# ZhiHuangHn/vtkCloudPoint

Hardware: AMD Instinct MI355X
Metric: Mpoints/s DBSCAN+label @10M pts (higher is better)
Workload: dtype f64; 1 GPU; C4: 10000000-pt cloud (half uniform background, 200 Gaussian blobs), one monolithic DBImproved.dbscan, metric L1_2D, eps 0.1, minPts 10; mode=single, points_total=10000000, points_per_gpu=10000000, clusters=27380, resident_in_hbm=True

## Files before the change

### vtkcloudpoint_amd/csrc/gridbuild.hip

```cpp
#include <algorithm>
#include <mutex>
#include <unordered_map>

#include "grid_common.hpp"

using namespace vcpg;

namespace {

constexpr int PT = 1024;
constexpr int PCH_MIN = 8192;
constexpr int FT = 1024;
constexpr uint32_t MAXB = 8192;
constexpr uint32_t wcap(int) { return 4096u; }
constexpr uint32_t QUEUE_FROM = 32;

typedef float4 Rec;

template <int GD>
__device__ __forceinline__ Rec rec_make(const float* qf, uint32_t idx, uint32_t cell) {
  return GD == 2 ? make_float4(qf[0], qf[1], __uint_as_float(idx), __uint_as_float(cell))
                 : make_float4(qf[0], qf[1], qf[2], __uint_as_float(idx));
}
template <int GD>
__device__ __forceinline__ uint32_t rec_cell(const Rec& r, const GridP& g, uint32_t& idx) {
  if (GD == 2) {
    idx = __float_as_uint(r.z);
    return __float_as_uint(r.w);
  }
  idx = __float_as_uint(r.w);
  const float qf[3] = {r.x, r.y, r.z};
  int cc[3];
  return cell_of32<3>(qf, g, cc);
}

template <int GD>
__device__ __forceinline__ uint32_t point_cell(const double* __restrict__ c, int64_t i, int stride, const GridP& g, float* qf) {
  double q[3];
  int cc[3];
  load_in<GD>(c, i, stride, q);
#pragma unroll
  for (int a = 0; a < GD; a++) qf[a] = rel32(q[a], g.mn[a], g.scale);
  return cell_of32<GD>(qf, g, cc);
}

struct PartGeom {
  uint32_t csh;
  uint32_t B;
  uint32_t a;
  uint32_t NS;
  uint32_t chunk;
  uint32_t nchunk;
};

inline int env_int(const char* name, int dflt, int lo, int hi) {
  const char* e = getenv(name);
  int v = e ? atoi(e) : dflt;
  return v < lo ? lo : v > hi ? hi : v;
}

inline PartGeom part_geom(int64_t n, uint32_t ncells) {
  static const int csh_max = env_int("VCP_CPB_LOG2", 14, 10, 14);
  static const int target = env_int("VCP_PART_CHUNKS", 256, 64, 8192);
  PartGeom p;
  int csh = csh_max;
  while (csh > 10 && ((uint64_t)ncells >> csh) * 4096ull < (uint64_t)n) csh--;
  p.csh = (uint32_t)csh;
  p.B = (uint32_t)((((uint64_t)ncells + 1) + ((1ull << p.csh) - 1)) >> p.csh);
  p.a = 0;
  while (((p.B + (1u << p.a) - 1u) >> p.a) > MAXB) p.a++;
  p.NS = (p.B + (1u << p.a) - 1u) >> p.a;
  int64_t chunk = (n + target - 1) / target;
  if (chunk < PCH_MIN) chunk = PCH_MIN;
  chunk = (chunk + PT - 1) / PT * PT;
  p.chunk = (uint32_t)chunk;
  p.nchunk = (uint32_t)((n + chunk - 1) / chunk);
  return p;
}

template <int GD, bool GROUPED>
__global__ __launch_bounds__(PT) void k_part_hist(const double* __restrict__ c, int64_t n, int stride, GridP g,
                                                 const int32_t* __restrict__ group, int glo, int ghi, uint32_t csh,
                                                 uint32_t B, uint32_t chunk, uint32_t nchunk,
                                                 uint32_t* __restrict__ counts, uint32_t* __restrict__ qcount,
                                                 uint32_t* __restrict__ ctcount) {
  extern __shared__ uint32_t h[];
  if (blockIdx.x == 0 && threadIdx.x == 0) {
    *qcount = 0u;
    ctcount[0] = 0u;
  }
  for (uint32_t k = threadIdx.x; k < B; k += PT) h[k] = 0;
  __syncthreads();
  const int64_t first = (int64_t)blockIdx.x * chunk;
  const int64_t last = min(first + (int64_t)chunk, n);
#pragma unroll 4
  for (int64_t i = first + threadIdx.x; i < last; i += PT) {
    if (GROUPED) {
      const int gg = group[i];
      if (gg < glo || gg >= ghi) continue;
    }
    float qf[3];
    atomicAdd(&h[point_cell<GD>(c, i, stride, g, qf) >> csh], 1u);
  }
  __syncthreads();
  for (uint32_t k = threadIdx.x; k < B; k += PT) counts[(size_t)k * nchunk + blockIdx.x] = h[k];
}

template <int GD, bool GROUPED>
__global__ __launch_bounds__(PT) void k_part_scatter(const double* __restrict__ c, int64_t n, int stride, GridP g,
                                                    const int32_t* __restrict__ group, int glo, int ghi, uint32_t csh,
                                                    uint32_t B, uint32_t chunk, uint32_t nchunk,
                                                    const uint32_t* __restrict__ base, Rec* __restrict__ rec,
                                                    uint32_t* __restrict__ pos) {
  extern __shared__ uint32_t h[];
  for (uint32_t k = threadIdx.x; k < B; k += PT) h[k] = base[(size_t)k * nchunk + blockIdx.x];
  __syncthreads();
  const int64_t first = (int64_t)blockIdx.x * chunk;
  const int64_t last = min(first + (int64_t)chunk, n);
#pragma unroll 4
  for (int64_t i = first + threadIdx.x; i < last; i += PT) {
    if (GROUPED) {
      const int gg = group[i];
      if (gg < glo || gg >= ghi) {
        if (pos) pos[i] = NONE;
        continue;
      }
    }
    float qf[3];
    const uint32_t cell = point_cell<GD>(c, i, stride, g, qf);
    rec[atomicAdd(&h[cell >> csh], 1u)] = rec_make<GD>(qf, (uint32_t)i, cell);
  }
}

__device__ __forceinline__ uint32_t padded(uint32_t i) { return i + (i >> 5); }

template <int GD, bool GROUPED, int NT = FT>
__device__ __forceinline__ void fine_flush(uint32_t s0, uint32_t m, const float* s32, const uint32_t* sidx,
                                           const uint32_t* __restrict__ ord, const uint8_t* __restrict__ in_classed,
                                           const int32_t* __restrict__ group, float* __restrict__ sorted32,
                                           uint32_t* __restrict__ sord, uint32_t* __restrict__ sidx_out,
                                           int32_t* __restrict__ sgroup, uint8_t* __restrict__ flags,
                                           uint32_t* __restrict__ pos) {
  if (GD == 2) {
    const float2* src = reinterpret_cast<const float2*>(s32);
    float2* dst = reinterpret_cast<float2*>(sorted32) + s0;
    for (uint32_t k = threadIdx.x; k < m; k += NT) dst[k] = src[k];
  } else {
    const float4* src = reinterpret_cast<const float4*>(s32);
    float4* dst = reinterpret_cast<float4*>(sorted32) + s0;
    for (uint32_t k = threadIdx.x; k < m; k += NT) dst[k] = src[k];
  }
  for (uint32_t k = threadIdx.x; k < m; k += NT) {
    const uint32_t i = sidx[k], p = s0 + k;
    sord[p] = ord ? ord[i] : i;
    if (sidx_out) sidx_out[p] = i;
    if (GROUPED) sgroup[p] = group[i];
    if (in_classed) flags[p] = in_classed[i] ? F_CLASSED : 0;
    if (pos) pos[i] = p;
  }
}

template <int GD>
__device__ __forceinline__ void stage_put(float* s32, uint32_t* sidx, uint32_t p, const Rec& r, uint32_t idx) {
  if (GD == 2) reinterpret_cast<float2*>(s32)[p] = make_float2(r.x, r.y);
  else reinterpret_cast<float4*>(s32)[p] = make_float4(r.x, r.y, r.z, 0.0f);
  sidx[p] = idx;
}

__device__ __forceinline__ void bucket_range(const uint32_t* __restrict__ bstart, uint32_t bstride, const uint32_t* __restrict__ total,
                                             uint32_t b, uint32_t B, uint32_t& s, uint32_t& e) {
  s = bstart[(size_t)b * bstride];
  e = (b + 1 < B) ? bstart[(size_t)(b + 1) * bstride] : *total;
}

template <int GD>
__global__ __launch_bounds__(FT) void k_part_split(const Rec* __restrict__ rec, Rec* __restrict__ rec2,
                                                  const uint32_t* __restrict__ base, const uint32_t* __restrict__ total,
                                                  uint32_t nchunk, uint32_t NS, uint32_t a, uint32_t csh, uint32_t B, GridP g,
                                                  uint32_t* __restrict__ bstart) {
  __shared__ uint32_t h[32];
  const uint32_t S = blockIdx.x;
  uint32_t s, e;
  bucket_range(base, nchunk, total, S, NS, s, e);
  const uint32_t subm = (1u << a) - 1u;
  if (threadIdx.x < 32) h[threadIdx.x] = 0u;
  __syncthreads();
  for (uint32_t j = s + threadIdx.x; j < e; j += FT) {
    uint32_t i;
    atomicAdd(&h[(rec_cell<GD>(rec[j], g, i) >> csh) & subm], 1u);
  }
  __syncthreads();
  if (threadIdx.x < 32) {
    const uint32_t v = h[threadIdx.x];
    uint32_t inc = v;
#pragma unroll
    for (int d = 1; d < 32; d <<= 1) {
      const uint32_t t = __shfl_up(inc, d, 64);
      if ((int)threadIdx.x >= d) inc += t;
    }
    const uint32_t first = s + inc - v;
    h[threadIdx.x] = first;
    const uint32_t bk = (S << a) + threadIdx.x;
    if (threadIdx.x <= subm && bk <= B) bstart[bk] = first;
  }
  __syncthreads();
  for (uint32_t j = s + threadIdx.x; j < e; j += FT) {
    const Rec r = rec[j];
    uint32_t i;
    rec2[atomicAdd(&h[(rec_cell<GD>(r, g, i) >> csh) & subm], 1u)] = r;
  }
}

constexpr int FS = 512;
constexpr uint32_t scap(int gd) { return gd == 2 ? 2048u : 1536u; }
constexpr uint32_t SPOP = 128;

template <int GD, bool GROUPED>
__global__ __launch_bounds__(FS) void k_part_fine_small(const Rec* __restrict__ rec, const uint32_t* __restrict__ bstart,
                                                       uint32_t bstride, const uint32_t* __restrict__ total, uint32_t B,
                                                       uint32_t csh, GridP g, const uint32_t* __restrict__ ord,
                                                       const uint8_t* __restrict__ in_classed, const int32_t* __restrict__ group,
                                                       uint4* __restrict__ ctwords, uint32_t* __restrict__ ctdense,
                                                       uint32_t* __restrict__ ctcount, uint8_t* __restrict__ bstate,
                                                       float* __restrict__ sorted32, uint32_t* __restrict__ sord,
                                                       uint32_t* __restrict__ sidx_out, int32_t* __restrict__ sgroup,
                                                       uint8_t* __restrict__ flags, uint32_t* __restrict__ pos) {
  constexpr uint32_t FPR = GD == 2 ? 2 : 4;
  constexpr uint32_t SCAP = scap(GD);
  constexpr int SRPT = SCAP / FS;
  __shared__ uint32_t ws[512 + 2];
  __shared__ uint32_t wlo[512], whi[512];
  __shared__ uint16_t wpi[512];
  __shared__ uint8_t sci[SCAP];
  __shared__ __attribute__((aligned(16))) uint16_t st32[SPOP][32];
  __shared__ __attribute__((aligned(16))) float s32[SCAP * FPR];
  __shared__ uint32_t sidx[SCAP];
  __shared__ uint32_t wsum[FS / 64];
  __shared__ uint32_t s_np, s_dbase;
  const uint32_t b = blockIdx.x;
  uint32_t s, e;
  bucket_range(bstart, bstride, total, b, B, s, e);
  const uint32_t m = e - s;
  if (b + 1 == B && threadIdx.x == 0) ctcount[1] = *total;
  if (m > SCAP) {
    if (threadIdx.x == 0) bstate[b] = 1;
    return;
  }
  const uint32_t CPB = 1u << csh, NW = CPB >> 5, c0 = b << csh;
  const int lane = threadIdx.x & 63, w = threadIdx.x >> 6;
  for (uint32_t k = threadIdx.x; k < NW + 1; k += FS) ws[k] = 0u;
  __syncthreads();
  Rec r[SRPT];
  uint32_t idx[SRPT], lw[SRPT], ci[SRPT], rnk[SRPT];
#pragma unroll
  for (int k = 0; k < SRPT; k++) {
    const uint32_t j = s + (uint32_t)k * FS + threadIdx.x;
    lw[k] = NONE;
    if (j < e) {
      r[k] = rec[j];
      const uint32_t c = rec_cell<GD>(r[k], g, idx[k]) - c0;
      lw[k] = c >> 5;
      ci[k] = c & 31u;
      rnk[k] = atomicAdd(&ws[lw[k]], 1u);
    }
  }
  __syncthreads();
  {
    const uint32_t v = threadIdx.x < NW ? ws[threadIdx.x] : 0u;
    uint32_t inc = v;
#pragma unroll
    for (int d = 1; d < 64; d <<= 1) {
      const uint32_t t = __shfl_up(inc, d, 64);
      if (lane >= d) inc += t;
    }
    if (lane == 63) wsum[w] = inc;
    __syncthreads();
    uint32_t pre = inc - v;
    for (int k = 0; k < w; k++) pre += wsum[k];
    if (threadIdx.x < NW) ws[threadIdx.x] = s + pre;
    if (threadIdx.x == 0) ws[NW] = e;
  }
  __syncthreads();
#pragma unroll
  for (int k = 0; k < SRPT; k++)
    if (lw[k] != NONE) sci[ws[lw[k]] - s + rnk[k]] = (uint8_t)ci[k];
  __syncthreads();
  bool popl = false;
  uint32_t lo = 0u, hi = 0u;
  if (threadIdx.x < NW) {
    const uint32_t a = ws[threadIdx.x] - s, k = ws[threadIdx.x + 1] - s - a;
    if (k > 64u) {
      popl = true;
    } else {
      for (uint32_t i = 0; i < k; i++) {
        const uint32_t bit = 1u << sci[a + i];
        if (lo & hi & bit) continue;
        if (lo & bit) hi ^= bit;
        lo ^= bit;
      }
      popl = (lo & hi) != 0u;
    }
  }
  {
    const unsigned long long dm = __ballot(popl);
    if (lane == 0) wsum[w] = (uint32_t)__popcll(dm);
    __syncthreads();
    uint32_t before = (uint32_t)__popcll(dm & ((1ull << lane) - 1ull)), tot = 0;
    for (int k = 0; k < FS / 64; k++) {
      if (k < w) before += wsum[k];
      tot += wsum[k];
    }
    if (threadIdx.x == 0) s_np = tot;
    if (threadIdx.x < NW) wpi[threadIdx.x] = popl ? (uint16_t)before : (uint16_t)0xFFFFu;
  }
  __syncthreads();
  const uint32_t np = s_np;
  if (np > SPOP) {
    if (threadIdx.x == 0) bstate[b] = 1;
    return;
  }
  if (threadIdx.x == 0) {
    bstate[b] = 0;
    s_dbase = np ? atomicAdd(&ctcount[0], np) : 0u;
  }
  for (uint32_t k = threadIdx.x; k < np * 16u; k += FS) reinterpret_cast<uint32_t*>(&st32[0][0])[k] = 0u;
  if (threadIdx.x < NW && !popl) {
    wlo[threadIdx.x] = lo;
    whi[threadIdx.x] = hi;
  }
  __syncthreads();
#pragma unroll
  for (int k = 0; k < SRPT; k++)
    if (lw[k] != NONE && wpi[lw[k]] != 0xFFFFu) {
      uint16_t* c = &st32[wpi[lw[k]]][ci[k]];
      atomicAdd(reinterpret_cast<uint32_t*>(reinterpret_cast<uintptr_t>(c) & ~(uintptr_t)3), ((uintptr_t)c & 2) ? 0x10000u : 1u);
    }
  __syncthreads();
  {
    const uint32_t hw = threadIdx.x >> 5, li = threadIdx.x & 31u;
    for (uint32_t wd = hw; wd < NW; wd += FS / 32) {
      const uint32_t pi = wpi[wd];
      if (pi == 0xFFFFu) continue;
      const uint32_t c = st32[pi][li];
      uint32_t inc = c;
#pragma unroll
      for (int d = 1; d < 32; d <<= 1) {
        const uint32_t t = __shfl_up(inc, d, 32);
        if ((int)li >= d) inc += t;
      }
      const uint32_t first = ws[wd] + inc - c;
      st32[pi][li] = (uint16_t)(first - s);
      ctdense[(size_t)(s_dbase + pi) * 32u + li] = first;
      const uint32_t cs = min(c, 3u);
      const unsigned long long blo = __ballot(cs & 1u), bhi = __ballot(cs >> 1);
      const int sh = (threadIdx.x & 32) ? 32 : 0;
      if (li == 0) {
        wlo[wd] = (uint32_t)(blo >> sh);
        whi[wd] = (uint32_t)(bhi >> sh);
      }
    }
  }
  __syncthreads();
#pragma unroll
  for (int k = 0; k < SRPT; k++) {
    if (lw[k] == NONE) continue;
    const uint32_t pi = wpi[lw[k]];
    uint32_t p;
    if (pi != 0xFFFFu) {
      uint16_t* c = &st32[pi][ci[k]];
      const bool up = ((uintptr_t)c & 2) != 0;
      const uint32_t old = atomicAdd(reinterpret_cast<uint32_t*>(reinterpret_cast<uintptr_t>(c) & ~(uintptr_t)3), up ? 0x10000u : 1u);
      p = up ? old >> 16 : old & 0xFFFFu;
    } else {
      const uint32_t l = wlo[lw[k]], h = whi[lw[k]], below = (1u << ci[k]) - 1u;
      const uint32_t a = ws[lw[k]] - s;
      p = a + (uint32_t)__popc(l & below) + 2u * (uint32_t)__popc(h & below);
      if ((h >> ci[k]) & 1u)
        for (uint32_t i = 0; i < rnk[k]; i++) p += sci[a + i] == (uint8_t)ci[k] ? 1u : 0u;
    }
    stage_put<GD>(s32, sidx, p, r[k], idx[k]);
  }
  if (threadIdx.x < NW) {
    const size_t W = (size_t)(c0 >> 5) + threadIdx.x;
    const uint32_t pi = wpi[threadIdx.x];
    if (W < vcp_ct_words(g.ncells))
      ctwords[W] = make_uint4(wlo[threadIdx.x], whi[threadIdx.x], ws[threadIdx.x], pi != 0xFFFFu ? s_dbase + pi : NONE);
  }
  __syncthreads();
  fine_flush<GD, GROUPED, FS>(s, m, s32, sidx, ord, in_classed, group, sorted32, sord, sidx_out, sgroup, flags, pos);
}

template <int GD, bool GROUPED>
__global__ __launch_bounds__(FT) void k_part_fine(const Rec* __restrict__ rec, uint32_t* __restrict__ rk,
                                                 const uint32_t* __restrict__ bstart, uint32_t bstride,
                                                 const uint32_t* __restrict__ total, uint32_t B, uint32_t csh, GridP g,
                                                 const uint32_t* __restrict__ ord, const uint8_t* __restrict__ in_classed,
                                                 const int32_t* __restrict__ group, uint4* __restrict__ ctwords,
                                                 uint32_t* __restrict__ ctdense, uint32_t* __restrict__ ctcount,
                                                 float* __restrict__ sorted32, uint32_t* __restrict__ sord,
                                                 uint32_t* __restrict__ sidx_out, int32_t* __restrict__ sgroup,
                                                 uint8_t* __restrict__ flags, uint32_t* __restrict__ pos,
                                                 uint2* __restrict__ queue, uint32_t* __restrict__ qcount,
                                                 const uint8_t* __restrict__ bstate) {
  extern __shared__ __attribute__((aligned(16))) unsigned char lds[];
  __shared__ uint32_t wsum[FT / 64];
  __shared__ uint32_t w_lo[512], w_hi[512], w_slot[512];
  __shared__ uint32_t s_dbase;
  const uint32_t b = blockIdx.x;
  if (bstate[b] == 0) return;
  constexpr uint32_t WCAP = wcap(GD);
  constexpr uint32_t FPR = GD == 2 ? 2 : 4;
  const uint32_t CPB = 1u << csh;
  uint32_t* cnt = reinterpret_cast<uint32_t*>(lds);
  float* s32 = reinterpret_cast<float*>(lds + (((size_t)padded(CPB) + 4) & ~3ull) * 4);
  uint32_t* sidx = reinterpret_cast<uint32_t*>(s32 + (size_t)WCAP * FPR);
  const uint32_t c0 = b << csh;
  uint32_t s, e;
  bucket_range(bstart, bstride, total, b, B, s, e);
  const uint32_t m = e - s;
  const bool big = m > WCAP;
  for (uint32_t k = threadIdx.x; k < padded(CPB); k += FT) cnt[k] = 0;
  __syncthreads();
  for (uint32_t j = s + threadIdx.x; j < e; j += FT) {
    uint32_t i;
    uint32_t* slot = &cnt[padded(rec_cell<GD>(rec[j], g, i) - c0)];
    if (big) rk[j] = atomicAdd(slot, 1u);
    else atomicAdd(slot, 1u);
  }
  __syncthreads();
  const uint32_t PER = CPB / FT;
  const uint32_t first = threadIdx.x * PER;
  uint32_t loc = 0;
  for (uint32_t k = 0; k < PER; k++) loc += cnt[padded(first + k)];
  const int lane = threadIdx.x & 63, w = threadIdx.x >> 6;
  uint32_t inc = loc;
#pragma unroll
  for (int d = 1; d < 64; d <<= 1) {
    const uint32_t t = __shfl_up(inc, d, 64);
    if (lane >= d) inc += t;
  }
  if (lane == 63) wsum[w] = inc;
  __syncthreads();
  uint32_t pre = s + inc - loc;
  for (int k = 0; k < w; k++) pre += wsum[k];
  const uint32_t NW = CPB >> 5;
  uint32_t plo = 0u, phi = 0u;
  const uint32_t wstart = pre;
  {
    const uint32_t bit0 = first & 31u;
    for (uint32_t k = 0; k < PER; k++) {
      const uint32_t v = cnt[padded(first + k)];
      cnt[padded(first + k)] = pre;
      pre += v;
      const uint32_t c = min(v, 3u);
      plo |= (c & 1u) << (bit0 + k);
      phi |= (c >> 1) << (bit0 + k);
    }
    for (uint32_t d = 1; d < 32u / PER; d <<= 1) {
      plo |= (uint32_t)__shfl_xor((int)plo, (int)d, 64);
      phi |= (uint32_t)__shfl_xor((int)phi, (int)d, 64);
    }
    if ((first & 31u) == 0u) {
      w_lo[first >> 5] = plo;
      w_hi[first >> 5] = phi;
      w_slot[first >> 5] = wstart;
    }
  }
  __syncthreads();
  {
    const bool popl = threadIdx.x < NW && (w_lo[threadIdx.x] & w_hi[threadIdx.x]) != 0u;
    const unsigned long long dm = __ballot(popl);
    if (lane == 0) wsum[w] = (uint32_t)__popcll(dm);
    __syncthreads();
    uint32_t before = (uint32_t)__popcll(dm & ((1ull << lane) - 1ull)), tot = 0;
    for (int k = 0; k < FT / 64; k++) {
      if (k < w) before += wsum[k];
      tot += wsum[k];
    }
    if (threadIdx.x == 0) s_dbase = tot ? atomicAdd(&ctcount[0], tot) : 0u;
    __syncthreads();
    if (threadIdx.x < NW) {
      const uint32_t slot = popl ? s_dbase + before : NONE;
      const uint32_t wpos = w_slot[threadIdx.x];
      w_slot[threadIdx.x] = slot;
      const size_t W = (size_t)(c0 >> 5) + threadIdx.x;
      if (W < vcp_ct_words(g.ncells))
        ctwords[W] = make_uint4(w_lo[threadIdx.x], w_hi[threadIdx.x], wpos, slot);
    }
    __syncthreads();
    const uint32_t hw = threadIdx.x >> 5, li = threadIdx.x & 31u;
    for (uint32_t j = hw; j < NW; j += FT / 32) {
      const uint32_t slot = w_slot[j];
      if (slot != NONE) ctdense[(size_t)slot * 32u + li] = cnt[padded(32u * j + li)];
    }
  }
  __syncthreads();
  if (!big) {
    for (uint32_t j = s + threadIdx.x; j < e; j += FT) {
      const Rec r = rec[j];
      uint32_t i;
      const uint32_t p = atomicAdd(&cnt[padded(rec_cell<GD>(r, g, i) - c0)], 1u) - s;
      stage_put<GD>(s32, sidx, p, r, i);
    }
    __syncthreads();
    fine_flush<GD, GROUPED>(s, m, s32, sidx, ord, in_classed, group, sorted32, sord, sidx_out, sgroup, flags, pos);
    return;
  }
  if (m > QUEUE_FROM * WCAP) {
    __shared__ uint32_t q0;
    const uint32_t nwin = (m + WCAP - 1) / WCAP;
    if (threadIdx.x == 0) q0 = atomicAdd(qcount, nwin);
    __syncthreads();
    for (uint32_t k = threadIdx.x; k < nwin; k += FT) queue[q0 + k] = make_uint2(b, k * WCAP);
    return;
  }
  for (uint32_t w0 = 0; w0 < m; w0 += WCAP) {
    for (uint32_t j = s + threadIdx.x; j < e; j += FT) {
      const Rec r = rec[j];
      uint32_t i;
      const uint32_t p = cnt[padded(rec_cell<GD>(r, g, i) - c0)] + rk[j] - s - w0;
      if (p < WCAP) stage_put<GD>(s32, sidx, p, r, i);
    }
    __syncthreads();
    fine_flush<GD, GROUPED>(s + w0, min(WCAP, m - w0), s32, sidx, ord, in_classed, group, sorted32, sord, sidx_out, sgroup,
                            flags, pos);
    __syncthreads();
  }
}

template <int GD, bool GROUPED>
__global__ __launch_bounds__(FT) void k_part_fine_windows(const Rec* __restrict__ rec, const uint32_t* __restrict__ rk,
                                                         const uint32_t* __restrict__ bstart, uint32_t bstride,
                                                         const uint32_t* __restrict__ total, uint32_t B, GridP g,
                                                         const uint32_t* __restrict__ ord, const uint8_t* __restrict__ in_classed,
                                                         const int32_t* __restrict__ group, CellTab ct,
                                                         float* __restrict__ sorted32,
                                                         uint32_t* __restrict__ sord, uint32_t* __restrict__ sidx_out,
                                                         int32_t* __restrict__ sgroup, uint8_t* __restrict__ flags,
                                                         uint32_t* __restrict__ pos, const uint2* __restrict__ queue,
                                                         const uint32_t* __restrict__ qcount) {
  extern __shared__ __attribute__((aligned(16))) unsigned char lds[];
  constexpr uint32_t WCAP = wcap(GD);
  constexpr uint32_t FPR = GD == 2 ? 2 : 4;
  float* s32 = reinterpret_cast<float*>(lds);
  uint32_t* sidx = reinterpret_cast<uint32_t*>(s32 + (size_t)WCAP * FPR);
  const uint32_t nq = *qcount;
  for (uint32_t qi = blockIdx.x; qi < nq; qi += gridDim.x) {
    const uint2 q = queue[qi];
    const uint32_t b = q.x, w0 = q.y;
    uint32_t s, e;
    bucket_range(bstart, bstride, total, b, B, s, e);
    const uint32_t m = e - s;
    for (uint32_t j = s + threadIdx.x; j < e; j += FT) {
      const Rec r = rec[j];
      uint32_t i;
      const uint32_t p = ct_start(ct, rec_cell<GD>(r, g, i)) + rk[j] - s - w0;
      if (p < WCAP) stage_put<GD>(s32, sidx, p, r, i);
    }
    __syncthreads();
    fine_flush<GD, GROUPED>(s + w0, min(WCAP, m - w0), s32, sidx, ord, in_classed, group, sorted32, sord, sidx_out, sgroup,
                            flags, pos);
    __syncthreads();
  }
}

constexpr int OT = 1024, OPT = 16;
constexpr int OWT = 512;

template <int OWSH>
__global__ __launch_bounds__(OT) void k_out_scatter(const uint32_t* __restrict__ sord, const uint32_t* __restrict__ labk,
                                                   int64_t n, uint32_t OB, uint32_t* __restrict__ gcur,
                                                   uint2* __restrict__ rec) {
  extern __shared__ uint32_t h[];
  for (uint32_t k = threadIdx.x; k < OB; k += OT) h[k] = 0;
  __syncthreads();
  const int64_t first = (int64_t)blockIdx.x * (OT * OPT);
  uint32_t o[OPT], w[OPT], r[OPT];
#pragma unroll
  for (int k = 0; k < OPT; k++) {
    const int64_t p = first + (int64_t)k * OT + threadIdx.x;
    o[k] = NONE;
    if (p < n) {
      o[k] = sord[p];
      w[k] = labk[p];
      r[k] = atomicAdd(&h[o[k] >> OWSH], 1u);
    }
  }
  __syncthreads();
  for (uint32_t k = threadIdx.x; k < OB; k += OT) {
    const uint32_t c = h[k];
    if (c) h[k] = atomicAdd(&gcur[k], c);
  }
  __syncthreads();
#pragma unroll
  for (int k = 0; k < OPT; k++) {
    if (o[k] == NONE) continue;
    const uint32_t bk = o[k] >> OWSH;
    rec[((size_t)bk << OWSH) + h[bk] + r[k]] = make_uint2(o[k], w[k]);
  }
}

template <int OWSH>
__global__ __launch_bounds__(OWT) void k_out_write(const uint2* __restrict__ rec, int64_t n, bool have_in_classed,
                                                  int32_t cf_in, int32_t* __restrict__ labels,
                                                  uint8_t* __restrict__ is_core, uint8_t* __restrict__ is_classed,
                                                  unsigned long long* __restrict__ counters, uint32_t* __restrict__ gcur) {
  extern __shared__ __attribute__((aligned(16))) uint32_t sw[];
  if (threadIdx.x == 0) gcur[blockIdx.x] = 0u;
  const int64_t lo = (int64_t)blockIdx.x << OWSH;
  const uint32_t cnt = (uint32_t)min((int64_t)1 << OWSH, n - lo);
  unsigned unclassed = 0;
  for (uint32_t j = threadIdx.x; j < cnt; j += OWT) {
    const uint2 v = rec[lo + j];
    sw[v.x - (uint32_t)lo] = v.y;
    if (!(v.y & 2u)) unclassed++;
  }
  __syncthreads();
  auto lab_of = [&](uint32_t w) { return (w >> 2) ? cf_in + (int32_t)(w >> 2) : 0; };
  auto core_of = [](uint32_t w) { return (uint32_t)((w & 3u) == 1u); };
  auto cls_of = [](uint32_t w) { return (uint32_t)((w & 2u) != 0u || (w >> 2) != 0u); };
  const bool vec = (((uintptr_t)labels & 15u) | ((uintptr_t)is_core & 3u) | ((uintptr_t)is_classed & 3u)) == 0;
  const uint32_t c4 = vec ? cnt >> 2 : 0u;
  for (uint32_t j = threadIdx.x; j < c4; j += OWT) {
    const uint4 w = reinterpret_cast<const uint4*>(sw)[j];
    const int4 l = make_int4(lab_of(w.x), lab_of(w.y), lab_of(w.z), lab_of(w.w));
    if (have_in_classed) {
      if (l.x) labels[lo + 4 * j] = l.x;
      if (l.y) labels[lo + 4 * j + 1] = l.y;
      if (l.z) labels[lo + 4 * j + 2] = l.z;
      if (l.w) labels[lo + 4 * j + 3] = l.w;
    } else {
      reinterpret_cast<int4*>(labels + lo)[j] = l;
    }
    if (is_core)
      reinterpret_cast<uint32_t*>(is_core + lo)[j] = core_of(w.x) | core_of(w.y) << 8 | core_of(w.z) << 16 | core_of(w.w) << 24;
    if (is_classed)
      reinterpret_cast<uint32_t*>(is_classed + lo)[j] = cls_of(w.x) | cls_of(w.y) << 8 | cls_of(w.z) << 16 | cls_of(w.w) << 24;
  }
  for (uint32_t j = (c4 << 2) + threadIdx.x; j < cnt; j += OWT) {
    const uint32_t w = sw[j];
    const int32_t l = lab_of(w);
    if (!have_in_classed || l) labels[lo + j] = l;
    if (is_core) is_core[lo + j] = (uint8_t)core_of(w);
    if (is_classed) is_classed[lo + j] = (uint8_t)cls_of(w);
  }
  if (have_in_classed) {
    __shared__ unsigned wc[OWT / 64];
#pragma unroll
    for (int d = 32; d > 0; d >>= 1) unclassed += __shfl_down(unclassed, d, 64);
    if ((threadIdx.x & 63) == 0) wc[threadIdx.x >> 6] = unclassed;
    __syncthreads();
    if (threadIdx.x == 0) {
      unsigned t = 0;
      for (int k = 0; k < OWT / 64; k++) t += wc[k];
      if (t) atomicAdd(&counters[CNT_UNCLASSED + (blockIdx.x & (CNT_SPREAD - 1))], (unsigned long long)t);
    }
  }
}

int allow_lds(vcp_ctx* ctx, const void* kernel, size_t bytes) {
  static std::mutex mu;
  static std::unordered_map<uint64_t, size_t> allowed;
  std::lock_guard<std::mutex> lk(mu);
  const uint64_t key = (uint64_t)reinterpret_cast<uintptr_t>(kernel) * 64u + (uint64_t)(ctx->device & 63);
  size_t& have = allowed.emplace(key, (size_t)64 * 1024).first->second;
  if (bytes > have) {
    VCP_HIP(ctx, hipFuncSetAttribute(kernel, hipFuncAttributeMaxDynamicSharedMemorySize, (int)bytes));
    have = bytes;
  }
  return VCP_OK;
}
template <class K>
int allow_lds(vcp_ctx* ctx, K kernel, size_t bytes) {
  return allow_lds(ctx, reinterpret_cast<const void*>(kernel), bytes);
}

template <int GD, bool GROUPED>
int build(vcp_ctx* ctx, const GridBuildArgs& a) {
  hipStream_t st = ctx->stream;
  const PartGeom pg = part_geom(a.n, a.g.ncells);
  const size_t nc = (size_t)pg.NS * pg.nchunk;
  VCP_TRY(vcp_ensure(ctx, ctx->b_hist, (nc + 8) * 4));
  VCP_TRY(vcp_ensure(ctx, ctx->b_rec, (size_t)a.n * sizeof(Rec)));
  uint32_t* counts = ctx->b_hist.as<uint32_t>();
  uint32_t* total = counts + nc;
  Rec* rec = ctx->b_rec.as<Rec>();
  const size_t lds_h = (size_t)pg.NS * 4;
  const uint32_t CPB = 1u << pg.csh;
  const size_t lds_f = ((((size_t)CPB + CPB / 32) + 4) & ~3ull) * 4 + (size_t)wcap(GD) * ((GD == 2 ? 8 : 16) + 4);
  VCP_TRY(allow_lds(ctx, k_part_fine<GD, GROUPED>, lds_f));
  VCP_TRY(vcp_ensure(ctx, ctx->b_fineq, ((size_t)a.n / wcap(GD) + pg.B + 8) * sizeof(uint2) + 64));
  uint32_t* qcount = ctx->b_fineq.as<uint32_t>();
  uint2* queue = reinterpret_cast<uint2*>(ctx->b_fineq.as<char>() + 64);
  vcp_phase(ctx, "part_hist");
  const uint32_t csh_a = pg.csh + pg.a;
  VCP_LAUNCH(ctx, (k_part_hist<GD, GROUPED>), dim3(pg.nchunk), dim3(PT), lds_h, st, a.d_coords, a.n, a.stride, a.g,
                  a.d_group, a.glo, a.ghi, csh_a, pg.NS, pg.chunk, pg.nchunk, counts, qcount, a.ctcount);
  VCP_TRY(vcp_exclusive_scan_u32(ctx, counts, counts, (int64_t)nc, total));
  vcp_phase(ctx, "part_scatter");
  VCP_LAUNCH(ctx, (k_part_scatter<GD, GROUPED>), dim3(pg.nchunk), dim3(PT), lds_h, st, a.d_coords, a.n, a.stride, a.g,
                  a.d_group, a.glo, a.ghi, csh_a, pg.NS, pg.chunk, pg.nchunk, counts, rec, a.pos);
  const uint32_t* bstart = counts;
  uint32_t bstride = pg.nchunk;
  if (pg.a > 0) {
    vcp_phase(ctx, "part_split");
    VCP_TRY(vcp_ensure(ctx, ctx->b_rec2, (size_t)a.n * sizeof(Rec)));
    VCP_TRY(vcp_ensure(ctx, ctx->b_bstart, ((size_t)pg.B + 2) * 4));
    VCP_LAUNCH(ctx, k_part_split<GD>, dim3(pg.NS), dim3(FT), 0, st, rec, ctx->b_rec2.as<Rec>(), counts, total, pg.nchunk,
                    pg.NS, pg.a, pg.csh, pg.B, a.g, ctx->b_bstart.as<uint32_t>());
    rec = ctx->b_rec2.as<Rec>();
    bstart = ctx->b_bstart.as<uint32_t>();
    bstride = 1;
  }
  vcp_phase(ctx, "part_fine");
  VCP_TRY(vcp_ensure(ctx, ctx->b_rank, (size_t)a.n * 4));
  VCP_TRY(vcp_ensure(ctx, ctx->b_bstate, (size_t)pg.B + 16));
  uint8_t* bstate = ctx->b_bstate.as<uint8_t>();
  VCP_LAUNCH(ctx, (k_part_fine_small<GD, GROUPED>), dim3(pg.B), dim3(FS), 0, st, rec, bstart, bstride, total, pg.B, pg.csh,
                  a.g, a.d_ord, a.d_in_classed, a.d_group, a.ctwords, a.ctdense, a.ctcount, bstate, a.sorted32, a.sord,
                  a.sidx, a.sgroup, a.flags, a.pos);
  VCP_LAUNCH(ctx, (k_part_fine<GD, GROUPED>), dim3(pg.B), dim3(FT), lds_f, st, rec, ctx->b_rank.as<uint32_t>(), bstart,
                  bstride, total, pg.B, pg.csh, a.g, a.d_ord, a.d_in_classed, a.d_group, a.ctwords, a.ctdense, a.ctcount,
                  a.sorted32, a.sord, a.sidx, a.sgroup, a.flags, a.pos, queue, qcount, bstate);
  {
    const size_t lds_w = (size_t)wcap(GD) * ((GD == 2 ? 8 : 16) + 4);
    VCP_TRY(allow_lds(ctx, k_part_fine_windows<GD, GROUPED>, lds_w));
    const unsigned gw = (unsigned)std::min<size_t>(768, (size_t)a.n / wcap(GD) + 1);
    const CellTab ct{a.ctwords, a.ctdense, a.ctcount + 1};
    VCP_LAUNCH(ctx, (k_part_fine_windows<GD, GROUPED>), dim3(gw), dim3(FT), lds_w, st, rec, ctx->b_rank.as<uint32_t>(),
                    bstart, bstride, total, pg.B, a.g, a.d_ord, a.d_in_classed, a.d_group, ct, a.sorted32,
                    a.sord, a.sidx, a.sgroup, a.flags, a.pos, queue, qcount);
  }
  return VCP_OK;
}

}

int vcp_grid_build_partition(vcp_ctx* ctx, const GridBuildArgs& a) {
  const bool grouped = a.d_group != nullptr;
  if (a.gd == 3) {
    if (grouped) return vcp_fail(ctx, VCP_ERR_ARG, "grouped calls are 2-D");
    return build<3, false>(ctx, a);
  }
  return grouped ? build<2, true>(ctx, a) : build<2, false>(ctx, a);
}

template <int OWSH>
static int output_partition(vcp_ctx* ctx, const GridOutputArgs& a) {
  hipStream_t st = ctx->stream;
  const uint32_t OB = (uint32_t)((a.n + (1 << OWSH) - 1) >> OWSH);
  const void* before = ctx->b_outcur.p;
  const size_t before_cap = ctx->b_outcur.cap;
  VCP_TRY(vcp_ensure(ctx, ctx->b_outcur, ((size_t)OB + 8) * 4));
  if (ctx->b_outcur.p != before || ctx->b_outcur.cap != before_cap)
    VCP_HIP(ctx, hipMemsetAsync(ctx->b_outcur.p, 0, ctx->b_outcur.cap, st));
  VCP_TRY(vcp_ensure(ctx, ctx->b_rec, (size_t)OB << (OWSH + 3)));
  uint32_t* gcur = ctx->b_outcur.as<uint32_t>();
  uint2* rec = ctx->b_rec.as<uint2>();
  VCP_TRY(allow_lds(ctx, k_out_write<OWSH>, (size_t)4 << OWSH));
  vcp_phase(ctx, "out_scatter");
  VCP_LAUNCH(ctx, k_out_scatter<OWSH>, dim3(vcp_blocks(a.n, OT * OPT)), dim3(OT), (size_t)OB * 4, st, a.sord, a.labk, a.n,
                  OB, gcur, rec);
  vcp_phase(ctx, "out_write");
  VCP_LAUNCH(ctx, k_out_write<OWSH>, dim3(OB), dim3(OWT), (size_t)4 << OWSH, st, rec, a.n, a.have_in_classed, a.cf_in,
                  a.labels, a.is_core, a.is_classed, a.counters, gcur);
  return VCP_OK;
}

int vcp_grid_output_partition(vcp_ctx* ctx, const GridOutputArgs& a) {
  if (a.n > ((int64_t)1 << 27)) return vcp_fail(ctx, VCP_ERR_TOO_LARGE, "more than 2^27 points: use the gather output");
  if (a.n >= ((int64_t)1 << 23)) return output_partition<15>(ctx, a);
  if (a.n >= ((int64_t)1 << 22)) return output_partition<14>(ctx, a);
  return output_partition<13>(ctx, a);
}
```

### vtkcloudpoint_amd/csrc/vcp_ctx.hpp

```cpp
#pragma once
#include <hip/hip_runtime.h>

#include <cstdarg>
#include <cstdint>
#include <cstdio>
#include <string>
#include <vector>

#include "vcp.h"

struct DevBuf {
  void* p = nullptr;
  size_t cap = 0;
  bool registered = false;
  template <class T>
  T* as() const { return reinterpret_cast<T*>(p); }
};

struct Phase {
  const char* name;
  hipEvent_t ev;
};

struct vcp_ctx {
  int device = 0;
  hipStream_t own_stream = nullptr;
  hipStream_t stream = nullptr;
  std::string err;
  hipDeviceProp_t prop;
  void* pinned = nullptr;
  size_t pinned_bytes = 0;
  void* stage = nullptr;
  size_t stage_bytes = 0;
  uint32_t scan_gen = 0;
  std::vector<DevBuf*> bufs;
  DevBuf b_cellof, b_rank, b_sidx, b_flags, b_parent, b_minord, b_seedflag,
      b_rootcl, b_clseed, b_scan_tmp, b_misc, b_in0, b_in1, b_in2, b_in3, b_out0, b_out1, b_out2,
      b_out3, b_icp_part, b_aux0, b_aux1, b_aux2, b_aux3, b_aux4, b_aux5, b_pos, b_labk, b_sgroup, b_wl, b_hist, b_rec, b_nn_misc, b_nn_cells, b_nn_cid, b_nn_rec, b_nn_cur, b_nbr, b_nboff, b_sorted32, b_self, b_outcur, b_fineq, b_rec2, b_bstart, b_ctw, b_ctd, b_bstate;
  DevBuf b_kd_in, b_kd_out, b_kd_outk, b_kd_part, b_kd_key, b_kd_val, b_kd_rec, b_kd_start, b_kd_heavy, b_kd_tmp;
  DevBuf b_sh_hull, b_sh_out, b_sh_flag;
  DevBuf b_mu_cent, b_mu_truth, b_mu_misc, b_mu_cell;
  DevBuf b_rg_in, b_rg_truth, b_rg_cell, b_rg_work;
  DevBuf b_et_in, b_et_out, b_et_kd, b_et_misc, b_et_cell, b_et_work, b_et_edge, b_et_tmp;
  DevBuf b_gd_in, b_gd_out, b_gd_misc, b_gd_cell, b_gd_work;
  DevBuf b_icpt;
  struct BlocksState* blocks = nullptr;
  struct SlabState* slab = nullptr;
  bool timing = false;
  std::vector<Phase> phases;
  std::vector<hipEvent_t> ev_pool;
  size_t ev_used = 0;
  std::vector<std::pair<const char*, float>> last_timing;
};

int vcp_fail(vcp_ctx* ctx, int code, const char* fmt, ...);
void* vcp_stage(vcp_ctx* ctx, size_t bytes);

#define VCP_HIP(ctx, call)                                                                    \
  do {                                                                                        \
    hipError_t e__ = (call);                                                                  \
    if (e__ != hipSuccess)                                                                    \
      return vcp_fail((ctx), VCP_ERR_HIP, "%s:%d %s -> %s", __FILE__, __LINE__, #call,        \
                      hipGetErrorString(e__));                                                \
  } while (0)

#define VCP_TRY(expr)        \
  do {                       \
    int rc__ = (expr);       \
    if (rc__ != VCP_OK) return rc__; \
  } while (0)

int vcp_ensure(vcp_ctx* ctx, DevBuf& b, size_t bytes, bool listed = true);
int vcp_bind(vcp_ctx* ctx);
void vcp_phase_reset(vcp_ctx* ctx);
void vcp_phase(vcp_ctx* ctx, const char* name);
int vcp_phase_finish(vcp_ctx* ctx);

constexpr unsigned vcp_blocks(int64_t n, int per_block, int cap = 1 << 30) {
  int64_t b = (n + per_block - 1) / per_block;
  if (b < 1) b = 1;
  if (b > cap) b = cap;
  return (unsigned)b;
}

constexpr bool vcp_launch_ok(dim3 grid, dim3 block, size_t lds) {
  return grid.x >= 1 && grid.y >= 1 && grid.z >= 1 && block.x >= 1 && block.y >= 1 && block.z >= 1 &&
         (uint64_t)grid.x * block.x <= 0xFFFFFFFFu && (uint64_t)grid.y * block.y <= 0xFFFFFFFFu &&
         (uint64_t)grid.z * block.z <= 0xFFFFFFFFu && block.x <= 1024 && block.y <= 1024 && block.z <= 1024 &&
         (uint64_t)block.x * block.y * block.z <= 1024 && lds <= 160 * 1024;
}
static_assert(vcp_launch_ok(dim3((1u << 24) - 1), dim3(256), 0) && !vcp_launch_ok(dim3(1u << 24), dim3(256), 0));
static_assert(vcp_launch_ok(dim3(1), dim3(1024), 0) && !vcp_launch_ok(dim3(1), dim3(1025), 0));
static_assert(vcp_launch_ok(dim3(1), dim3(64), 163840) && !vcp_launch_ok(dim3(1), dim3(64), 163841));
static_assert(!vcp_launch_ok(dim3(0), dim3(64), 0) && !vcp_launch_ok(dim3(1, 1, 0), dim3(64), 0) &&
                  !vcp_launch_ok(dim3(1), dim3(64, 0), 0));

#define VCP_LAUNCH(ctx, kernel, grid, block, lds, stream, ...)                                                         \
  do {                                                                                                                 \
    const dim3 g__ = (grid), b__ = (block);                                                                            \
    const size_t l__ = (lds);                                                                                          \
    if (!vcp_launch_ok(g__, b__, l__))                                                                                 \
      return vcp_fail((ctx), VCP_ERR_TOO_LARGE, "%s: grid %ux%ux%u, block %ux%ux%u, lds %zu", #kernel, g__.x, g__.y,   \
                      g__.z, b__.x, b__.y, b__.z, l__);                                                                \
    hipLaunchKernelGGL(kernel, g__, b__, l__, stream, __VA_ARGS__);                                                    \
    const hipError_t e__ = hipGetLastError();                                                                          \
    if (e__ != hipSuccess) return vcp_fail((ctx), VCP_ERR_HIP, "%s: %s", #kernel, hipGetErrorString(e__));             \
  } while (0)

int vcp_exclusive_scan_u32(vcp_ctx* ctx, const uint32_t* d_in, uint32_t* d_out, int64_t n,
                           uint32_t* d_total);
int vcp_exclusive_max_scan_u32(vcp_ctx* ctx, const uint32_t* d_in, uint32_t* d_out, int64_t n,
                           uint32_t* d_total);
```

Before: 7014 Mpoints/s.

## Size output windows to CU count and make scatter blocks persistent

Result: no change. 7052 Mpoints/s (median of 6 runs) (+0.5%).

```diff
diff --git a/vtkcloudpoint_amd/csrc/gridbuild.hip b/vtkcloudpoint_amd/csrc/gridbuild.hip
--- a/vtkcloudpoint_amd/csrc/gridbuild.hip
+++ b/vtkcloudpoint_amd/csrc/gridbuild.hip
@@ -566,49 +566,54 @@
 
 constexpr int OT = 1024, OPT = 16;
 constexpr int OWT = 512;
-
-template <int OWSH>
+constexpr uint32_t OW_MAX = 1u << 15, OW_MIN = 1u << 13;
+constexpr size_t OW_TAIL = 4 * (OWT / 64);
+static_assert(OW_MAX <= VCP_DIV_MAX_D && ((uint64_t)1 << 27) + OW_MAX <= VCP_DIV_MAX_O, "windows and positions vcp_div covers");
+
 __global__ __launch_bounds__(OT) void k_out_scatter(const uint32_t* __restrict__ sord, const uint32_t* __restrict__ labk,
-                                                   int64_t n, uint32_t OB, uint32_t* __restrict__ gcur,
-                                                   uint2* __restrict__ rec) {
+                                                   uint32_t n, uint32_t share, VcpDiv wd, uint32_t OB,
+                                                   uint32_t* __restrict__ gcur, uint2* __restrict__ rec) {
   extern __shared__ uint32_t h[];
-  for (uint32_t k = threadIdx.x; k < OB; k += OT) h[k] = 0;
-  __syncthreads();
-  const int64_t first = (int64_t)blockIdx.x * (OT * OPT);
-  uint32_t o[OPT], w[OPT], r[OPT];
-#pragma unroll
-  for (int k = 0; k < OPT; k++) {
-    const int64_t p = first + (int64_t)k * OT + threadIdx.x;
-    o[k] = NONE;
-    if (p < n) {
-      o[k] = sord[p];
-      w[k] = labk[p];
-      r[k] = atomicAdd(&h[o[k] >> OWSH], 1u);
-    }
-  }
-  __syncthreads();
-  for (uint32_t k = threadIdx.x; k < OB; k += OT) {
-    const uint32_t c = h[k];
-    if (c) h[k] = atomicAdd(&gcur[k], c);
-  }
-  __syncthreads();
-#pragma unroll
-  for (int k = 0; k < OPT; k++) {
-    if (o[k] == NONE) continue;
-    const uint32_t bk = o[k] >> OWSH;
-    rec[((size_t)bk << OWSH) + h[bk] + r[k]] = make_uint2(o[k], w[k]);
-  }
-}
-
-template <int OWSH>
-__global__ __launch_bounds__(OWT) void k_out_write(const uint2* __restrict__ rec, int64_t n, bool have_in_classed,
+  const uint32_t lo = blockIdx.x * share;
+  const uint32_t hi = min(n, lo + share);
+  for (uint32_t first = lo; first < hi; first += OT * OPT) {
+    for (uint32_t k = threadIdx.x; k < OB; k += OT) h[k] = 0;
+    __syncthreads();
+    uint32_t o[OPT], w[OPT], r[OPT];
+#pragma unroll
+    for (int k = 0; k < OPT; k++) {
+      const uint32_t p = first + (uint32_t)k * OT + threadIdx.x;
+      o[k] = NONE;
+      if (p < hi) {
+        o[k] = sord[p];
+        w[k] = labk[p];
+        r[k] = atomicAdd(&h[vcp_div(o[k], wd)], 1u);
+      }
+    }
+    __syncthreads();
+    for (uint32_t k = threadIdx.x; k < OB; k += OT) {
+      const uint32_t c = h[k];
+      if (c) h[k] = atomicAdd(&gcur[k], c);
+    }
+    __syncthreads();
+#pragma unroll
+    for (int k = 0; k < OPT; k++) {
+      if (o[k] == NONE) continue;
+      const uint32_t bk = vcp_div(o[k], wd);
+      rec[(size_t)bk * wd.d + h[bk] + r[k]] = make_uint2(o[k], w[k]);
+    }
+    __syncthreads();
+  }
+}
+
+__global__ __launch_bounds__(OWT) void k_out_write(const uint2* __restrict__ rec, int64_t n, uint32_t W, bool have_in_classed,
                                                   int32_t cf_in, int32_t* __restrict__ labels,
                                                   uint8_t* __restrict__ is_core, uint8_t* __restrict__ is_classed,
                                                   unsigned long long* __restrict__ counters, uint32_t* __restrict__ gcur) {
   extern __shared__ __attribute__((aligned(16))) uint32_t sw[];
   if (threadIdx.x == 0) gcur[blockIdx.x] = 0u;
-  const int64_t lo = (int64_t)blockIdx.x << OWSH;
-  const uint32_t cnt = (uint32_t)min((int64_t)1 << OWSH, n - lo);
+  const int64_t lo = (int64_t)blockIdx.x * W;
+  const uint32_t cnt = (uint32_t)min((int64_t)W, n - lo);
   unsigned unclassed = 0;
   for (uint32_t j = threadIdx.x; j < cnt; j += OWT) {
     const uint2 v = rec[lo + j];
@@ -645,7 +650,7 @@
     if (is_classed) is_classed[lo + j] = (uint8_t)cls_of(w);
   }
   if (have_in_classed) {
-    __shared__ unsigned wc[OWT / 64];
+    uint32_t* wc = sw + W;
 #pragma unroll
     for (int d = 32; d > 0; d >>= 1) unclassed += __shfl_down(unclassed, d, 64);
     if ((threadIdx.x & 63) == 0) wc[threadIdx.x >> 6] = unclassed;
@@ -745,31 +750,56 @@
   return grouped ? build<2, true>(ctx, a) : build<2, false>(ctx, a);
 }
 
-template <int OWSH>
+static uint32_t out_write_per_cu(const vcp_ctx* ctx, uint32_t W) {
+  const size_t lds = (((size_t)4 * W + OW_TAIL) + 2047) & ~(size_t)2047;
+  const uint32_t by_lds = (uint32_t)((size_t)160 * 1024 / lds);
+  const uint32_t by_threads = (uint32_t)std::max(1, ctx->prop.maxThreadsPerMultiProcessor / OWT);
+  return std::max(1u, std::min(by_lds, by_threads));
+}
+
+static uint32_t out_window(const vcp_ctx* ctx, int64_t n) {
+  const uint32_t cus = (uint32_t)std::max(1, ctx->prop.multiProcessorCount);
+  for (uint32_t m = 1;; m++) {
+    const int64_t ob_want = (int64_t)m * cus;
+    const uint32_t W = (uint32_t)std::max<int64_t>(OW_MIN, ((n + ob_want - 1) / ob_want + 3) & ~(int64_t)3);
+    if (W > OW_MAX) continue;
+    const uint32_t ob = (uint32_t)((n + W - 1) / W), held = cus * out_write_per_cu(ctx, W);
+    if (ob <= held || ob % held == 0 || W == OW_MIN) return W;
+  }
+}
+
 static int output_partition(vcp_ctx* ctx, const GridOutputArgs& a) {
   hipStream_t st = ctx->stream;
-  const uint32_t OB = (uint32_t)((a.n + (1 << OWSH) - 1) >> OWSH);
+  if (!ctx->out_scatter_wgs) {
+    int per_cu = 0;
+    VCP_HIP(ctx, hipOccupancyMaxActiveBlocksPerMultiprocessor(&per_cu, k_out_scatter, OT, (size_t)4 * 1024));
+    ctx->out_scatter_wgs = (uint32_t)std::max(1, per_cu) * (uint32_t)std::max(1, ctx->prop.multiProcessorCount);
+  }
+  const uint32_t W = out_window(ctx, a.n);
+  const VcpDiv wd = vcp_div_make(W);
+  const uint32_t OB = (uint32_t)((a.n + W - 1) / W);
+  const uint32_t G = ctx->out_scatter_wgs;
+  const uint32_t share = std::max<uint32_t>(OT * OPT / 4, (uint32_t)(((a.n + G - 1) / G + 63) & ~(int64_t)63));
   const void* before = ctx->b_outcur.p;
   const size_t before_cap = ctx->b_outcur.cap;
   VCP_TRY(vcp_ensure(ctx, ctx->b_outcur, ((size_t)OB + 8) * 4));
   if (ctx->b_outcur.p != before || ctx->b_outcur.cap != before_cap)
     VCP_HIP(ctx, hipMemsetAsync(ctx->b_outcur.p, 0, ctx->b_outcur.cap, st));
-  VCP_TRY(vcp_ensure(ctx, ctx->b_rec, (size_t)OB << (OWSH + 3)));
+  VCP_TRY(vcp_ensure(ctx, ctx->b_rec, (size_t)OB * W * sizeof(uint2)));
   uint32_t* gcur = ctx->b_outcur.as<uint32_t>();
   uint2* rec = ctx->b_rec.as<uint2>();
-  VCP_TRY(allow_lds(ctx, k_out_write<OWSH>, (size_t)4 << OWSH));
+  const size_t lds_w = (size_t)4 * W + OW_TAIL;
+  VCP_TRY(allow_lds(ctx, k_out_write, lds_w));
   vcp_phase(ctx, "out_scatter");
-  VCP_LAUNCH(ctx, k_out_scatter<OWSH>, dim3(vcp_blocks(a.n, OT * OPT)), dim3(OT), (size_t)OB * 4, st, a.sord, a.labk, a.n,
-                  OB, gcur, rec);
+  VCP_LAUNCH(ctx, k_out_scatter, dim3(vcp_blocks(a.n, (int)share)), dim3(OT), (size_t)OB * 4, st, a.sord, a.labk,
+                  (uint32_t)a.n, share, wd, OB, gcur, rec);
   vcp_phase(ctx, "out_write");
-  VCP_LAUNCH(ctx, k_out_write<OWSH>, dim3(OB), dim3(OWT), (size_t)4 << OWSH, st, rec, a.n, a.have_in_classed, a.cf_in,
-                  a.labels, a.is_core, a.is_classed, a.counters, gcur);
+  VCP_LAUNCH(ctx, k_out_write, dim3(OB), dim3(OWT), lds_w, st, rec, a.n, W, a.have_in_classed, a.cf_in, a.labels,
+                  a.is_core, a.is_classed, a.counters, gcur);
   return VCP_OK;
 }
 
 int vcp_grid_output_partition(vcp_ctx* ctx, const GridOutputArgs& a) {
   if (a.n > ((int64_t)1 << 27)) return vcp_fail(ctx, VCP_ERR_TOO_LARGE, "more than 2^27 points: use the gather output");
-  if (a.n >= ((int64_t)1 << 23)) return output_partition<15>(ctx, a);
-  if (a.n >= ((int64_t)1 << 22)) return output_partition<14>(ctx, a);
-  return output_partition<13>(ctx, a);
-}
+  return output_partition(ctx, a);
+}
diff --git a/vtkcloudpoint_amd/csrc/vcp_ctx.hpp b/vtkcloudpoint_amd/csrc/vcp_ctx.hpp
--- a/vtkcloudpoint_amd/csrc/vcp_ctx.hpp
+++ b/vtkcloudpoint_amd/csrc/vcp_ctx.hpp
@@ -44,6 +44,7 @@
   DevBuf b_et_in, b_et_out, b_et_kd, b_et_misc, b_et_cell, b_et_work, b_et_edge, b_et_tmp;
   DevBuf b_gd_in, b_gd_out, b_gd_misc, b_gd_cell, b_gd_work;
   DevBuf b_icpt;
+  uint32_t out_scatter_wgs = 0;
   struct BlocksState* blocks = nullptr;
   struct SlabState* slab = nullptr;
   bool timing = false;
@@ -95,6 +96,31 @@
 static_assert(!vcp_launch_ok(dim3(0), dim3(64), 0) && !vcp_launch_ok(dim3(1, 1, 0), dim3(64), 0) &&
                   !vcp_launch_ok(dim3(1), dim3(64, 0), 0));
 
+struct VcpDiv {
+  uint32_t d, mul, sh;
+};
+constexpr uint32_t VCP_DIV_MAX_D = 1u << 15, VCP_DIV_MAX_O = 1u << 30;
+constexpr VcpDiv vcp_div_make(uint32_t d) {
+  uint32_t sh = 0;
+  while ((2u << sh) < d) sh++;
+  return VcpDiv{d, (uint32_t)(((uint64_t)1 << (32 + sh)) / d) + 1u, sh};
+}
+__host__ __device__ constexpr uint32_t vcp_div(uint32_t o, const VcpDiv& v) {
+  return (uint32_t)(((uint64_t)o * v.mul) >> 32) >> v.sh;
+}
+constexpr bool vcp_div_selfcheck() {
+  for (uint32_t d = 4; d <= VCP_DIV_MAX_D; d += 4) {
+    const VcpDiv v = vcp_div_make(d);
+    const uint32_t top = (VCP_DIV_MAX_O - 1) / d * d;
+    if ((uint64_t)v.mul * d <= ((uint64_t)1 << (32 + v.sh))) return false;
+    if (vcp_div(0, v) != 0 || vcp_div(d - 1, v) != 0 || vcp_div(d, v) != 1) return false;
+    if (vcp_div(top - 1, v) != top / d - 1 || vcp_div(top, v) != top / d) return false;
+    if (vcp_div(VCP_DIV_MAX_O - 1, v) != (VCP_DIV_MAX_O - 1) / d) return false;
+  }
+  return true;
+}
+static_assert(vcp_div_selfcheck(), "the multiply-high division is not exact over its range");
+
 #define VCP_LAUNCH(ctx, kernel, grid, block, lds, stream, ...)                                                         \
   do {                                                                                                                 \
     const dim3 g__ = (grid), b__ = (block);                                                                            \
```
